# coolo/rl-6-nimmt

Hardware: AMD Instinct MI355X
Metric: env-steps/sec at 65536 concurrent 4-player games, 1/2/4/8 MI355X (higher is better)
Workload: dtype u32; 1 GPU; config2: 65536 x 4-player DrunkHamster self-play per GPU, one episode (10 env-steps) per launch, numpy-MT RNG, int8 obs + actions + rewards + done emitted; games_per_gpu=65536, players=4, env_steps_per_launch=655360, rng=numpy, obs=True, parallelism=dp1 (independent game shards, no data-path collective), launches_per_call=4

## Files before the change

### include/sechs.h

```cpp
#ifndef SECHS_H
#define SECHS_H
#include <stddef.h>
#include <stdint.h>

#ifdef __cplusplus
extern "C" {
#endif

typedef struct sn_env sn_env;

typedef enum {
    SN_OK = 0,
    SN_EINVAL = 1,
    SN_EHIP = 2,
    SN_ENOMEM = 3,
    SN_EUNSUPPORTED = 4,
    SN_ERNG = 5,
} sn_status;

enum {
    SN_RNG_PHILOX = 0,
    SN_RNG_NUMPY_MT = 1,
};

// ... 12 lines not shown
sn_status sn_destroy(sn_env* env);
sn_status sn_info(const sn_env* env, int64_t* num_games, int* num_players, int* num_cards, int* rng_mode);

sn_status sn_reset(sn_env* env, const uint8_t* decks, void* stream);

sn_status sn_reset_to(sn_env* env, const int8_t* board, const int8_t* hands, void* stream);

sn_status sn_step(sn_env* env, const int32_t* actions, int32_t* rewards, uint8_t* done, int32_t* invalid, int flags,
                  void* stream);

sn_status sn_rollout(sn_env* env, int steps, int32_t* rewards, uint8_t* done, uint8_t* actions, int8_t* obs,
                     int obs_stride, int flags, void* stream);

sn_status sn_obs(sn_env* env, void* obs, int dtype, int obs_stride, int flags, void* stream);
sn_status sn_hands(sn_env* env, int8_t* hands, void* stream);
sn_status sn_board(sn_env* env, int8_t* board, void* stream);
sn_status sn_scores(sn_env* env, int32_t* scores, void* stream);
sn_status sn_results(sn_env* env, int32_t* sum_results, int32_t* episodes, void* stream);
sn_status sn_clear_results(sn_env* env, void* stream);

sn_status sn_mt_get(sn_env* env, int64_t game, uint32_t* key_host, int32_t* pos_host);
sn_status sn_mt_set(sn_env* env, int64_t game, const uint32_t* key_host, int32_t pos);
sn_status sn_philox_counter(sn_env* env, int64_t game, uint64_t* counter_host);

int64_t sn_state_bytes(int64_t num_games, int num_players, int rng_mode, int league, int64_t* header_bytes,
                       int64_t* record_bytes);
int64_t sn_state_size(const sn_env* env);
sn_status sn_state_save(sn_env* env, void* blob, int64_t blob_bytes, void* stream);
sn_status sn_state_load(sn_env* env, const void* blob, int64_t blob_bytes, int64_t first, void* stream);

enum { SN_OPT_RING_WORDS = 1, SN_OPT_CHUNK_STEPS = 2, SN_OPT_PIPELINE = 3, SN_OPT_TIMING = 4, SN_OPT_PIPE_GPW = 5,
       SN_OPT_PIPE_LEAD = 6, SN_OPT_PLAY_SPLIT = 7, SN_OPT_PLAY_QUAD = 8, SN_OPT_TWIST_ROUND = 9,
       SN_OPT_TWIST_EVERY = 10, SN_OPT_PIPE_FUSED = 11, SN_OPT_TWIST_SKIP = 12, SN_OPT_PIPE_DEC = 13,
       SN_OPT_TWIST_DEPTH = 14, SN_OPT_PLAY_GROUP = 15, SN_OPT_DEC_WALK = 16, SN_OPT_DEC_EARLY = 17 };
sn_status sn_set_option(sn_env* env, int option, int value);
sn_status sn_pipe_errors(sn_env* env, uint32_t* count);
sn_status sn_kernel_times(sn_env* env, float* play_ms, float* ahead_ms, int32_t* n);
sn_status sn_kernel_times_dec(sn_env* env, float* play_ms, float* ahead_ms, float* decode_ms, int32_t* n);
sn_status sn_debug_phases(uint64_t* out, int n);
sn_status sn_debug_puct_phases(uint64_t* out, int n);
sn_status sn_debug_pipe_words(sn_env* env, int what, int slot, uint32_t* out);
sn_status sn_debug_failures(uint32_t* count, uint32_t* first_line, int selftest);

sn_status sn_step1(sn_env* env, const int32_t* actions_host, int32_t* out_host, int flags);
sn_status sn_reset1(sn_env* env, const uint32_t* key_host, int32_t pos, uint32_t* key_out_host, int32_t* pos_out,
                    int32_t* out_host, int flags);

sn_status sn_league_config(sn_env* env, int num_agents, int min_players, int max_players);
sn_status sn_league_rollout(sn_env* env, int steps, int32_t* rewards, uint8_t* done, uint8_t* actions, int8_t* obs,
                            int obs_stride, int32_t* records, void* stream);
sn_status sn_league_seats(sn_env* env, uint32_t* out, void* stream);

enum { SN_AGENT_RANDOM = 0, SN_AGENT_MCS = 1, SN_AGENT_EXTERNAL = 2 };
sn_status sn_league_agents(sn_env* env, const int32_t* kinds_host, const int32_t* mc_per_card_host,
                           const int32_t* mc_max_host);
sn_status sn_league_step(sn_env* env, const int32_t* actions, int32_t* rewards, int32_t* played, int32_t* records,
                         int32_t* invalid, int32_t* status, void* stream);
sn_status sn_elo_replay(const int32_t* records_host, int64_t num_games, int max_players, int num_agents, double elo_k,
                        double* elos_host);


sn_status sn_mcs_memorize(sn_env* env, uint32_t* avail, int mcs_num_cards, void* stream);

sn_status sn_mcs_rollouts(sn_env* env, const uint32_t* avail, int rollouts, uint64_t seed, uint32_t decision_step,
                          int32_t* sums, void* stream);
sn_status sn_mcs_rollouts_ex(sn_env* env, const uint32_t* avail, int rollouts, uint64_t seed, uint32_t decision_step,
                             int32_t* sums, int32_t* playouts, void* stream);
// ... 101 lines not shown
```

### rl-6-nimmt_amd/csrc/sechs_env.hip

```cpp
#include <hip/hip_runtime.h>

#include <cmath>
#include <cstdio>
#include <cstdlib>
#include <cstring>
#include <new>
#include <string>
#include <type_traits>

#define SECHS_DEBUG_HERE
#include "sechs_state.h"

using namespace sechs;

#include "sechs_reset.h"
#include "sechs_mt_ahead.h"
#include "sechs_play.h"
#include "sechs_decode.h"
#include "sechs_env1.h"
#include "sechs_play_split.h"

template <typename T>
__global__ void k_obs(DevState s, T* out, int stride, int summ) {
    const int64_t i = (int64_t)blockIdx.x * blockDim.x + threadIdx.x;
// ... 127 lines not shown
    DevState& s = e->s;
    s.B = num_games, s.N = num_players, s.C = num_cards, s.rng_mode = rng_mode;
    s.seed = seed, s.game_offset = game_offset;
    const int64_t B = num_games, N = num_players;
    struct {
        void** p;
        size_t bytes;
    } allocs[] = {
        {(void**)&s.hand, sizeof(uint32_t) * N * 3 * B},   {(void**)&s.row_lo, sizeof(uint32_t) * kRows * B},
        {(void**)&s.row_hi, sizeof(uint32_t) * kRows * B}, {(void**)&s.score, sizeof(int32_t) * N * B},
        {(void**)&s.sum_res, sizeof(int32_t) * N * B},     {(void**)&s.episodes, sizeof(int32_t) * B},
        {(void**)&s.mt_pos, sizeof(uint32_t) * B},         {(void**)&s.ctr, sizeof(uint64_t) * B},
        {(void**)&s.mt, rng_mode == SN_RNG_NUMPY_MT ? sizeof(uint32_t) * kMtN * B : 4},
        {(void**)&s.mt0, sizeof(uint32_t) * kMt0Levels * B},
    };
    for (auto& a : allocs) {
        if (hipMalloc(a.p, a.bytes) != hipSuccess) {
            sn_destroy(e);
            return fail(SN_ENOMEM, "hipMalloc of device state failed");
        }
        (void)hipMemset(*a.p, 0, a.bytes);
    }
    e->opt.chunk_steps = 10;
    e->opt.pipe = 1;
    e->opt.pipe_gpw = 64;
    e->opt.pipe_lead = kPipeLead;
    e->phase = -1;
    e->opt.play_split = 1;
    e->opt.twist_round = 1;
    e->opt.twist_every = 4;
    env_default("SECHS_TWIST_EVERY", 1, kTwistEveryMax, e->opt.twist_every);
    e->opt.twist_depth = 3;
    env_default("SECHS_TWIST_DEPTH", 0, kTwistDepthMax, e->opt.twist_depth);
    e->opt.pipe_serial = 0;
    env_default("SECHS_PIPE_SERIAL", 0, 1, e->opt.pipe_serial);
    e->opt.play_group = 1;
    env_default("SECHS_PLAY_GROUP", 0, 1, e->opt.play_group);
    e->opt.dec_walk = 1;
    env_default("SECHS_DEC_WALK", 0, 1, e->opt.dec_walk);
    e->opt.dec_early = 1;
    env_default("SECHS_DEC_EARLY", 0, 1, e->opt.dec_early);
    e->opt.pipe_dec = 1;
    env_default("SECHS_PIPE_DEC", 0, 1, e->opt.pipe_dec);
    if (rng_mode == SN_RNG_NUMPY_MT) {
        struct {
            void** p;
            size_t bytes;
        } pal[] = {{(void**)&s.pring, (size_t)kPipeRing * B},
                   {(void**)&s.pabsc, sizeof(uint32_t) * (kPipeSlots + 2) * B},
                   {(void**)&s.ptend, sizeof(uint32_t) * kPipeSlots * B}, {(void**)&s.ptp, sizeof(uint32_t) * B},
                   {(void**)&s.perr, sizeof(uint32_t)},
                   {(void**)&s.drec, N <= kSplitMaxPlayers ? sizeof(u32x4) * kDecRecords * kDecQuads * B : 16}};
        for (auto& a : pal) {
            if (hipMalloc(a.p, a.bytes) != hipSuccess) {
                sn_destroy(e);
                return fail(SN_ENOMEM, "hipMalloc of the MT pipeline failed");
            }
            (void)hipMemset(*a.p, 0, a.bytes);
        }
        int sysfence = 0;
        env_default("SECHS_EV_SYSFENCE", 0, 1, sysfence);
        const unsigned evf = hipEventDisableTiming | (sysfence ? 0u : (unsigned)hipEventDisableSystemFence);
        if (hipStreamCreateWithFlags(&e->pl.side, hipStreamNonBlocking) != hipSuccess ||
            hipStreamCreateWithFlags(&e->pl.side2, hipStreamNonBlocking) != hipSuccess ||
            hipEventCreateWithFlags(&e->pl.ev_prep2, evf) != hipSuccess ||
            hipEventCreateWithFlags(&e->pl.ev_prep, evf) != hipSuccess ||
            hipEventCreateWithFlags(&e->pl.ev_main, evf) != hipSuccess ||
            hipEventCreateWithFlags(&e->pl.ev_play, evf) != hipSuccess) {
// ... 82 lines not shown
            if (s.ring) (void)hipFree(s.ring);
            s.ring = nullptr;
            s.ring_w = 0;
            if (value) {
                if (hipMalloc((void**)&s.ring, (size_t)value * (size_t)s.B) != hipSuccess) return fail(SN_ENOMEM, "ring allocation failed");
                s.ring_w = value;
            }
            return SN_OK;
        }
        case SN_OPT_CHUNK_STEPS:
            if (value < 1) return fail(SN_EINVAL, "chunk steps must be >= 1");
            e->opt.chunk_steps = value;
            return SN_OK;
        case SN_OPT_PIPELINE:
            if (value != 0 && value != 1) return fail(SN_EINVAL, "pipeline must be 0 or 1");
            e->opt.pipe = value;
            return SN_OK;
        case SN_OPT_PIPE_GPW:
            if (value != 32 && value != 64) return fail(SN_EINVAL, "games per wave must be 32 or 64");
            e->opt.pipe_gpw = value;
            return SN_OK;
        case SN_OPT_PLAY_SPLIT:
            if (value < 0 || value > 1) return fail(SN_EINVAL, "play split must be 0 or 1");
            e->opt.play_split = value;
            return SN_OK;
        case SN_OPT_TWIST_EVERY:
            if (value < 1 || value > kTwistEveryMax) return fail(SN_EINVAL, "twist every must be 1 .. 5");
            e->opt.twist_every = value;
            return SN_OK;
        case SN_OPT_TWIST_DEPTH:
            if (value < 0 || value > kTwistDepthMax) return fail(SN_EINVAL, "twist depth must be 0 .. 3");
            e->opt.twist_depth = value;
            return SN_OK;
        case SN_OPT_TWIST_ROUND:
            if (value < 0 || value > 1) return fail(SN_EINVAL, "twist round must be 0 or 1");
            e->opt.twist_round = value;
            return SN_OK;
        case SN_OPT_PLAY_QUAD:
        case SN_OPT_PIPE_FUSED:
            return fail(SN_EUNSUPPORTED, "option removed (k_play_quad / the fused twist measured slower)");
        case SN_OPT_PIPE_DEC:
            if (value < 0 || value > 1) return fail(SN_EINVAL, "pipe dec must be 0 or 1");
            e->opt.pipe_dec = value;
            return SN_OK;
        case SN_OPT_PLAY_GROUP:
            if (value < 0 || value > 1) return fail(SN_EINVAL, "play group must be 0 or 1");
            e->opt.play_group = value;
            return SN_OK;
        case SN_OPT_DEC_WALK:
            if (value < 0 || value > 1) return fail(SN_EINVAL, "dec walk must be 0 or 1");
            e->opt.dec_walk = value;
            return SN_OK;
        case SN_OPT_DEC_EARLY:
            if (value < 0 || value > 1) return fail(SN_EINVAL, "dec early must be 0 or 1");
            e->opt.dec_early = value;
            return SN_OK;
        case SN_OPT_TWIST_SKIP:
            if (value < 0 || value > 1) return fail(SN_EINVAL, "twist skip must be 0 or 1");
            e->opt.twist_skip = value;
            return SN_OK;
        case SN_OPT_PIPE_LEAD:
            if (value < 64 || value > kPipeLead) return fail(SN_EINVAL, "pipe lead must be in 64..600");
            e->opt.pipe_lead = value;
            return SN_OK;
        case SN_OPT_TIMING:
            if (value < 0 || value > 4096) return fail(SN_EINVAL, "timing launches must be in 0..4096");
// ... 159 lines not shown
        return SN_OK;
    }
    return launch_play_mode(s, a, mode, 64, st);
}

constexpr uint64_t kStartUp = ~0ull;
constexpr uint32_t kSlotMask = (uint32_t)kPipeSlots - 1u;
static inline int pabsc_in(uint64_t p) { return (int)((p + kSlotMask) & kSlotMask); }
static inline int pabsc_out(uint64_t p) { return (int)(p & kSlotMask); }
static inline int ptend_slot(uint64_t G) { return (int)(G & 1u); }
static inline int dec_slot(uint64_t G) { return kDecSlot + (int)(G & 1u); }
static inline int dec_record(int64_t episode) { return (int)(episode % kDecRecords); }

sn_status sn_pipe_sync(sn_env* e, hipStream_t st) {
    if (!e || !e->pl.valid) return SN_OK;
    HIP_TRY(hipStreamWaitEvent(st, e->pl.ev_play, 0));
    HIP_TRY(hipEventRecord(e->pl.ev_prep, e->pl.side));
    HIP_TRY(hipStreamWaitEvent(st, e->pl.ev_prep, 0));
    HIP_TRY(hipEventRecord(e->pl.ev_prep2, e->pl.side2));
    HIP_TRY(hipStreamWaitEvent(st, e->pl.ev_prep2, 0));
    hipLaunchKernelGGL(k_pipe_code, dim3((unsigned)((e->s.B + kBlock / 64 - 1) / (kBlock / 64))), dim3(kBlock), 0, st,
                       e->s, e->pl.pl_cout, e->pl.tw_out);
    HIP_TRY(hipGetLastError());
    e->pl.valid = 0;
    return SN_OK;
}

static int pipe_max_chunk(int N) { return N <= 4 ? 10 : 5; }

static sn_status launch_ahead(const DevState& s, bool init, bool round_tw, const AheadArgs& aa, hipStream_t st) {
    const dim3 pg((unsigned)((s.B + kBlock / 64 - 1) / (kBlock / 64)));
    if (init && round_tw) hipLaunchKernelGGL((k_mt_ahead<true, true>), pg, dim3(kBlock), 0, st, s, aa);
    else if (init) hipLaunchKernelGGL((k_mt_ahead<true, false>), pg, dim3(kBlock), 0, st, s, aa);
    else if (round_tw) hipLaunchKernelGGL((k_mt_ahead<false, true>), pg, dim3(kBlock), 0, st, s, aa);
    else hipLaunchKernelGGL((k_mt_ahead<false, false>), pg, dim3(kBlock), 0, st, s, aa);
    HIP_TRY(hipGetLastError());
    return SN_OK;
}

static sn_status dec_launch(sn_env* e, int64_t e0, int ne, int phi0, int tpar, int cin, int cout, hipStream_t st) {
    const DevState& s = e->s;
    const DecArgs d{dec_record(e0), ne, phi0, tpar, cin, cout};
    const dim3 grid((unsigned)((s.B + kDecBlock - 1) / kDecBlock));
    SN_DISPATCH_N(s.N, {
        if constexpr (NN <= kSplitMaxPlayers) {
            const bool walk = e->opt.dec_walk != 0;
            const bool touch = e->opt.dec_early != 0;
            if (walk && touch) hipLaunchKernelGGL((k_decode<NN, true, true>), grid, dim3(kDecBlock), 0, st, s, d);
            else if (walk) hipLaunchKernelGGL((k_decode<NN, true, false>), grid, dim3(kDecBlock), 0, st, s, d);
            else if (touch) hipLaunchKernelGGL((k_decode<NN, false, true>), grid, dim3(kDecBlock), 0, st, s, d);
            else hipLaunchKernelGGL((k_decode<NN, false, false>), grid, dim3(kDecBlock), 0, st, s, d);
        }
    });
    HIP_TRY(hipGetLastError());
    return SN_OK;
}

static bool dec_ok(const sn_env* e, const PlayArgs& a) {
    return e->opt.pipe_dec && e->phase >= 0 && (a.flags & SN_AUTO_RESET) && !a.actions && !a.invalid && !e->s.lg_K &&
           e->s.N <= kSplitMaxPlayers && e->opt.pipe_gpw == 64 && e->s.drec;
}

static sn_status pipe_start(sn_env* e, int K, bool dec, int lead, hipStream_t st) {
    sn_env::Pipeline& pl = e->pl;
    const AheadArgs aa{dec ? dec_slot(kStartUp - 1) : pabsc_out(kStartUp), ptend_slot(kStartUp - 1), ptend_slot(kStartUp), lead,
                       e->perr_host_dev, dec ? pabsc_out(kStartUp) : -1, e->opt.twist_depth};
    pl.tw_out = ptend_slot(kStartUp), pl.pl_cout = pabsc_out(kStartUp), pl.launches = 0;
    if (const sn_status r = launch_ahead(e->s, true, e->opt.twist_round, aa, st); r != SN_OK) return r;
    if (dec) {
        pl.dec_e = 0;
        const sn_status r = dec_launch(e, 0, K + 1, e->phase, ptend_slot(kStartUp), dec_slot(kStartUp - 1), dec_slot(kStartUp), st);
        if (r != SN_OK) return r;
        pl.dec_next = K + 1;
    }
    HIP_TRY(hipEventRecord(pl.ev_prep, st));
    pl.valid = 1, pl.K = K, pl.dec = dec ? 1 : 0;
    return SN_OK;
}

static sn_status pipe_twist(sn_env* e, uint64_t G, uint64_t p, int64_t e_start, int lead, int ti, hipStream_t st) {
    sn_env::Pipeline& pl = e->pl;
    hipEvent_t* tv = (ti >= 0) ? e->tev + kTimingEvents * ti : nullptr;
    if (e->opt.pipe_serial) HIP_TRY(hipEventRecord(pl.ev_main, st));
    HIP_TRY(hipStreamWaitEvent(pl.side, pl.ev_main, 0));
    if (tv) HIP_TRY(hipEventRecord(tv[2], pl.side));
    const AheadArgs aa{pl.dec ? dec_slot(G - 1) : pabsc_in(p), ptend_slot(G - 1), ptend_slot(G),
                       (e->opt.twist_skip && G >= 1u) ? 0 : lead, e->perr_host_dev, -1, e->opt.twist_depth};
    if (const sn_status r = launch_ahead(e->s, false, e->opt.twist_round, aa, pl.side); r != SN_OK) return r;
    if (tv) HIP_TRY(hipEventRecord(tv[3], pl.side));
    if (pl.dec) {
        const int64_t target = e_start + 2 * pl.K + 1;
        if (e->opt.pipe_serial || G == 0u) HIP_TRY(hipStreamWaitEvent(pl.side2, pl.ev_main, 0));
        if (G >= 1u) HIP_TRY(hipStreamWaitEvent(pl.side2, pl.evt[ptend_slot(G - 1)], 0));
        if (tv) HIP_TRY(hipEventRecord(tv[4], pl.side2));
        const int ne = target > pl.dec_next ? (int)(target - pl.dec_next) : 0;
        const sn_status r = dec_launch(e, pl.dec_next, ne, 0, ptend_slot(G - 1), dec_slot(G - 1), dec_slot(G), pl.side2);
        if (r != SN_OK) return r;
        pl.dec_next = max(pl.dec_next, target);
        if (tv) {
            HIP_TRY(hipEventRecord(tv[5], pl.side2));
            e->tev_tw[ti] |= 2;
        }
        HIP_TRY(hipEventRecord(pl.evd[ptend_slot(G)], pl.side2));
    }
    HIP_TRY(hipEventRecord(pl.evt[ptend_slot(G)], pl.side));
    HIP_TRY(hipEventRecord(pl.ev_prep, pl.side));
    pl.tw_out = ptend_slot(G);
    return SN_OK;
}

static sn_status launch_pipe(sn_env* e, PlayArgs a, LdsPlan plan, hipStream_t st) {
    const DevState& s = e->s;
    sn_env::Pipeline& pl = e->pl;
    const int gpw = e->opt.pipe_gpw, K = e->opt.twist_every;
    const bool dec = dec_ok(e, a);
    const int mode = dec ? RNG_NUMPY_DEC : RNG_NUMPY_PIPE;
    apply_plan(a, dec ? lds_plan(s.N, obs_staged(a.obs, a.obs_stride), RNG_NUMPY_DEC) : plan);
    if (pl.valid && (pl.K != K || (pl.dec != 0) != dec)) {
        if (const sn_status r = sn_pipe_sync(e, st); r != SN_OK) return r;
    }
    const int lead = dec ? min(e->opt.pipe_lead * (K + 1), kPipeRing - kMtN) : e->opt.pipe_lead * K;
    static_assert(kPipeLeadMax <= kPipeRing - kMtN, "the decode-ahead lead is never capped by the ring");
    if (!pl.valid) {
        if (const sn_status r = pipe_start(e, K, dec, lead, st); r != SN_OK) return r;
    } else {
// ... 472 lines not shown
```

### rl-6-nimmt_amd/csrc/sechs_mt_ahead.h

```cpp
#pragma once

constexpr int kPrepGamesPerWave = 4;

template <int NB, int GPW>
__global__ __launch_bounds__(kBlock) void k_mt_prep(DevState s) {
    constexpr uint32_t W = 64u * NB;
    constexpr uint32_t D = kMtN - kMtM;
    const int64_t g0 = ((int64_t)blockIdx.x * (kBlock / 64) + (threadIdx.x >> 6)) * GPW;
    if (g0 >= s.B) return;
    const uint32_t lane = threadIdx.x & 63u;
    uint32_t rem[GPW], KT[GPW], T0[GPW], base[GPW];
    uint32_t A[GPW][NB + 1], C[GPW][NB + 1];
    const uint32_t codes = (lane < (uint32_t)GPW) ? s.mt_pos[min(g0 + (int64_t)lane, s.B - 1)] : 0u;
#pragma unroll
    for (int q = 0; q < GPW; q++) {
        const int64_t g = min(g0 + q, s.B - 1);
        const uint32_t code = __builtin_amdgcn_readlane(codes, q);
        const uint32_t T = code & 0x7FFu;
        rem[q] = (code >> 16) & kMtCntMask;
        const uint32_t add = (rem[q] >= W) ? 0u : ((W - rem[q] + 7u) & ~7u);
        KT[q] = rem[q] + add;
        T0[q] = (T == (uint32_t)kMtN) ? 0u : T;
        base[q] = T0[q] + kMtN - rem[q];
        const uint32_t* st = s.mt + g * kMtN;
// ... 59 lines not shown
                        const uint32_t keep = (1u << (8u * (r + D - k))) - 1u;
                        *dst = (*dst & keep) | (d & ~keep);
                    }
                }
            }
        }
        if (lane == 0u && kt > r) {
            const uint32_t Tn = T0[q] + (kt - r);
            s.mt_pos[g] = ((Tn > (uint32_t)kMtN) ? Tn - kMtN : Tn) | (kt << 16);
        }
    }
}

#ifndef SECHS_NT_OBS
#define SECHS_NT_OBS 1
#endif
#ifndef SECHS_NT_MORE
#define SECHS_NT_MORE 1
#endif
template <class T>
__device__ __forceinline__ void st_nt(T* p, T v, bool nt) {
    if (nt) __builtin_nontemporal_store(v, p);
    else *p = v;
}

struct AheadArgs {
    int cin;
    int tin;
    int tout;
    int lead;
    uint32_t* perr_mirror;
    int cin_copy;
    int depth;
};

__device__ __forceinline__ void mt_round_load(const DevState& s, int64_t G, uint32_t lane, uint32_t (&v)[10]) {
    const uint32_t* st = s.mt + G * kMtN;
#pragma unroll
    for (int k = 0; k < 10; k++) {
        const uint32_t i = 64u * k + lane;
        v[k] = (i < (uint32_t)kMtN) ? st[i] : 0u;
    }
}

__device__ __forceinline__ void mt_round_to_lds(uint32_t lane, uint32_t* w, const uint32_t (&v)[10]) {
#pragma unroll
    for (int k = 0; k < 10; k++) {
        const uint32_t i = 64u * k + lane;
        if (i < (uint32_t)kMtN) w[i] = v[k];
    }
    __builtin_amdgcn_fence(__ATOMIC_SEQ_CST, "wavefront");
}

__device__ __forceinline__ uint32_t mt_twist_lds(uint32_t lane, uint32_t* w) {
    constexpr uint32_t D = kMtN - kMtM;
    const uint32_t old0 = (uint32_t)__builtin_amdgcn_readfirstlane((int)w[0]);
    uint32_t nv[4];
#pragma unroll
    for (int k = 0; k < 4; k++) {
        const uint32_t i = 64u * k + lane;
        nv[k] = (i < D) ? mt_mix(w[i], w[i + 1u], w[i + kMtM]) : 0u;
    }
    __builtin_amdgcn_fence(__ATOMIC_SEQ_CST, "wavefront");
#pragma unroll
    for (int k = 0; k < 4; k++) {
        const uint32_t i = 64u * k + lane;
// ... 24 lines not shown
        if (i < (uint32_t)kMtN) w[i] = nv[k];
    }
    __builtin_amdgcn_fence(__ATOMIC_SEQ_CST, "wavefront");
    return old0;
}

__device__ __forceinline__ void mt_round_emit(const DevState& s, int64_t G, uint32_t lane, const uint32_t* w,
                                              uint32_t te) {
    uint8_t* ring = (uint8_t*)s.pring;
#pragma unroll
    for (int k = 0; k < 3; k++) {
        const uint32_t d = 64u * k + lane;
        if (d < (uint32_t)kMtN / 4u) {
            const u32x4 x = *(const u32x4*)(w + 4u * d);
            const uint32_t y = (mt_temper(x.x) & 0xFFu) | ((mt_temper(x.y) & 0xFFu) << 8) |
                               ((mt_temper(x.z) & 0xFFu) << 16) | ((mt_temper(x.w) & 0xFFu) << 24);
            const uint32_t ri = (te + 4u * d) & (uint32_t)(kPipeRing - 1);
            st_nt((uint32_t*)(ring + ring_byte(ri, G, s.B)), y, SECHS_NT_MORE);
        }
    }
    __builtin_amdgcn_fence(__ATOMIC_SEQ_CST, "wavefront");
}

__device__ __forceinline__ void mt_round_store(const DevState& s, int64_t G, uint32_t lane, const uint32_t* w) {
    uint32_t* st = s.mt + G * kMtN;
#pragma unroll
    for (int k = 0; k < 10; k++) {
        const uint32_t i = 64u * k + lane;
        if (i < (uint32_t)kMtN) st_nt(&st[i], w[i], SECHS_NT_MORE);
    }
    __builtin_amdgcn_fence(__ATOMIC_SEQ_CST, "wavefront");
}

template <bool INIT, bool ROUND = false>
__global__ __launch_bounds__(kBlock) void k_mt_ahead(DevState s, AheadArgs a) {
    constexpr uint32_t D = kMtN - kMtM;
    constexpr uint32_t P1 = 224;
    const int64_t g = (int64_t)blockIdx.x * (kBlock / 64) + (threadIdx.x >> 6);
    if (g >= s.B) return;
    const uint32_t lane = threadIdx.x & 63u;
    const int64_t B = s.B;
    if (g == 0 && lane == 0u && a.perr_mirror)
        __hip_atomic_store(a.perr_mirror, __hip_atomic_load(s.perr, __ATOMIC_RELAXED, __HIP_MEMORY_SCOPE_AGENT),
                           __ATOMIC_RELAXED, __HIP_MEMORY_SCOPE_SYSTEM);
    uint32_t* st = s.mt + g * kMtN;
    uint8_t* ring = (uint8_t*)s.pring;
    uint32_t Tp, t0, c;
    if (INIT) {
        const uint32_t code = s.mt_pos[g];
        Tp = code & 0x7FFu;
        const uint32_t rem = (code >> 16) & kMtCntMask;
        t0 = 0u;
        c = 0u - rem;
        for (uint32_t k0 = 0; k0 < rem; k0 += 64u) {
            const uint32_t k = k0 + lane;
            if (k < rem) {
                const uint32_t v = st[(Tp + kMtN - rem + k) % (uint32_t)kMtN];
                const uint32_t ri = (c + k) & (uint32_t)(kPipeRing - 1);
                ring[ring_byte(ri, g, B)] = (uint8_t)(mt_temper(v) & 0xFFu);
            }
        }
        if (lane == 0u) {
            s.pabsc[(int64_t)a.cin * B + g] = c;
            if (a.cin_copy >= 0) s.pabsc[(int64_t)a.cin_copy * B + g] = c;
        }
    } else {
        Tp = s.ptp[g];
        t0 = s.ptend[(int64_t)a.tin * B + g];
        c = s.pabsc[(int64_t)a.cin * B + g];
    }
    const int32_t lead = (int32_t)(t0 - c);
    if (lead < 0 && lane == 0u) atomicAdd(s.perr, 1u);
    const uint32_t T0 = (Tp == (uint32_t)kMtN) ? 0u : Tp;
    const int32_t lo = a.lead + ((ROUND && INIT) ? kMtN * (int32_t)(g % (int64_t)(a.depth + 1)) : 0);
    const int32_t hi = (ROUND && !INIT) ? a.lead + kMtN * a.depth : lo;
    const bool refill = lead >= 0 && lead < lo;
    const uint32_t n = ROUND ? ((refill && T0 != 0u) ? (uint32_t)kMtN - T0 : 0u)
                             : ((lead >= 0 && lead < a.lead) ? (((uint32_t)(a.lead - lead)) & ~7u) : 0u);
    auto ring_dword = [&](uint32_t j, uint32_t v) {
        const uint32_t y = mt_temper(v) & 0xFFu;
        const uint32_t d = y | (__shfl_down(y, 1) << 8) | (__shfl_down(y, 2) << 16) | (__shfl_down(y, 3) << 24);
        const uint32_t ri = (t0 + j) & (uint32_t)(kPipeRing - 1);
        if ((lane & 3u) == 0u && j < n) st_nt((uint32_t*)(ring + ring_byte(ri, g, B)), d, SECHS_NT_MORE);
    };
    uint32_t ncross = 0u, old0 = 0u;
    auto cross = [&](bool hit, uint32_t old) {
        const uint64_t m = __ballot(hit);
        if (m) {
            const uint32_t v = __shfl(old, (int)__builtin_ctzll(m));
            const uint32_t up = __shfl_up(old0, 1);
            old0 = lane ? up : v;
            ncross++;
        }
    };
    uint32_t A[4] = {0u, 0u, 0u, 0u}, Bv[4], Cv[4], IX[4];
#pragma unroll
    for (int b = 0; b < 4; b++) {
        const uint32_t j = 64u * b + lane;
        IX[b] = 0xFFFFu;
        if (j < n && j < P1) {
            const uint32_t idx = (T0 + j) % (uint32_t)kMtN;
            IX[b] = idx;
            A[b] = st[idx];
            Bv[b] = st[(idx + 1u == (uint32_t)kMtN) ? 0u : idx + 1u];
            Cv[b] = st[(idx < D) ? idx + kMtM : idx - D];
        }
    }
#pragma unroll
// ... 15 lines not shown
        if (j < n) {
            const uint32_t idx = (T0 + j) % (uint32_t)kMtN;
            aa = st[idx];
            v = mt_mix(aa, st[(idx + 1u == (uint32_t)kMtN) ? 0u : idx + 1u], st[(idx < D) ? idx + kMtM : idx - D]);
            st[idx] = v;
            at0 = idx == 0u;
        }
        cross(at0, aa);
        ring_dword(j, v);
    }
    uint32_t Tn = Tp, te = t0 + n;
    if (n) {
        Tn = T0 + n;
        while (Tn > (uint32_t)kMtN) Tn -= kMtN;
    }
    if constexpr (ROUND) {
        if (refill && lead + (int32_t)(te - t0) < hi) {
            __shared__ __attribute__((aligned(16))) uint32_t wround[kBlock / 64][kMtN];
            uint32_t* w = wround[threadIdx.x >> 6];
            __builtin_amdgcn_fence(__ATOMIC_SEQ_CST, "wavefront");
            uint32_t v[10];
            mt_round_load(s, g, lane, v);
            mt_round_to_lds(lane, w, v);
            for (int rr = 0; rr < kMt0Levels - 1 && lead + (int32_t)(te - t0) < hi; rr++) {
                cross(true, mt_twist_lds(lane, w));
                mt_round_emit(s, g, lane, w, te);
                te += kMtN;
            }
            mt_round_store(s, g, lane, w);
            Tn = kMtN;
        }
    }
    SN_DASSERT(ncross <= (uint32_t)kMt0Levels);
    SN_DASSERT(lead < 0 || te - c <= (uint32_t)kPipeSpanMax);
    SN_DASSERT(!ROUND || lead < 0 || te == t0 || (int32_t)(te - c) >= hi);
    SN_DASSERT(!ROUND || te == t0 || Tn == (uint32_t)kMtN);
    if (lane == 0u) {
        s.ptp[g] = Tn;
        s.ptend[(int64_t)a.tout * B + g] = te;
    }
    if (ncross) {
        const uint32_t stk = (lane < (uint32_t)kMt0Levels) ? s.mt0[g * kMt0Levels + lane] : 0u;
        const uint32_t older = __shfl(stk, (int)((lane - ncross) & 63u));
        if (lane < (uint32_t)kMt0Levels) s.mt0[g * kMt0Levels + lane] = (lane < ncross) ? old0 : older;
    }
}

__device__ __forceinline__ uint32_t mt_untwist_y_dev(uint32_t t) {
    const uint32_t lsb = t >> 31;
    return (((lsb ? (t ^ 0x9908b0dfu) : t)) << 1) | lsb;
}

__global__ __launch_bounds__(kBlock) void k_pipe_code(DevState s, int cin, int tin) {
    const int64_t g = (int64_t)blockIdx.x * (kBlock / 64) + (threadIdx.x >> 6);
    if (g >= s.B) return;
    const uint32_t lane = threadIdx.x & 63u;
    int32_t rem = (int32_t)(s.ptend[(int64_t)tin * s.B + g] - s.pabsc[(int64_t)cin * s.B + g]);
    if (rem < 0 && lane == 0u) atomicAdd(s.perr, 1u);
    uint32_t tp = s.ptp[g];
    __shared__ uint32_t sw[kBlock / 64][kMtN], sy[kBlock / 64][kMtN];
    uint32_t* w = sw[threadIdx.x >> 6];
    uint32_t* y = sy[threadIdx.x >> 6];
    uint32_t* a = s.mt + g * kMtN;
    constexpr uint32_t D = kMtN - kMtM;
    int lvl = 0;
    const uint32_t code0 = s.mt_pos[g];
    const bool at0 = code0 == ((uint32_t)kMtN | ((uint32_t)kMtN << 16)) &&
// ... 37 lines not shown
```

### rl-6-nimmt_amd/csrc/sechs_state.h

```cpp
#pragma once
#include <hip/hip_runtime.h>

#include <string>

#include "../../include/sechs.h"
#include "sechs_device.h"

namespace sechs {

struct DevState {
    int64_t B;
    int N, C, rng_mode, pad_;
    uint64_t seed, game_offset;
    uint32_t* hand;
    uint32_t* row_lo;
    uint32_t* row_hi;
    int32_t* score;
    int32_t* sum_res;
    int32_t* episodes;
    uint32_t* mt;
    uint32_t* mt_pos;
    uint64_t* ctr;
    uint32_t* mt0;
    u32x4* ring;
// ... 2 lines not shown
    u32x4* pring;
    uint32_t* pabsc;
    uint32_t* ptend;
    uint32_t* ptp;
    uint32_t* perr;
    u32x4* drec;
    uint32_t* lgs;
    int lg_K, lg_lo, lg_hi, lg_pad;
    uint32_t* lmem;
    int32_t* lpc;
    int32_t* lpf;
};

constexpr int kMt0Levels = 16;
constexpr int kPipeSlots = 8;
constexpr int kDecSlot = kPipeSlots;
constexpr int kDecRecords = 16;
constexpr int kDecQuads = 6;
constexpr int kTimingEvents = 6;
constexpr int kPipeRing = 8192;

__host__ __device__ __forceinline__ int64_t ring16(uint32_t u, int64_t g, int64_t B) {
    u &= (uint32_t)(kPipeRing / 16 - 1);
    return ((int64_t)(u >> 2) * B + g) * 4 + (u & 3u);
}
__host__ __device__ __forceinline__ int64_t ring_byte(uint32_t ri, int64_t g, int64_t B) {
    return ring16(ri >> 4, g, B) * 16 + (ri & 15u);
}

constexpr int kPipeLead = 600;
constexpr int kPipeWin = 240;

constexpr int kTwistEveryMax = 5, kTwistDepthMax = 3;
static_assert((kPipeSlots & (kPipeSlots - 1)) == 0, "pabsc / ptend slots are taken mod kPipeSlots with a mask");
static_assert(kPipeSlots >= kTwistEveryMax + 3, "no play launch overwrites a pabsc slot a running twist reads");
static_assert(kDecRecords >= 3 * kTwistEveryMax + 1, "no decode overwrites a record a running play launch reads");
constexpr int kPipeLeadMax = kPipeLead * (kTwistEveryMax + 1);
constexpr int kPipeSpanMax = kPipeLeadMax + kMtN * kTwistDepthMax + kMtN - 1;
static_assert(kPipeSpanMax + 64 <= kPipeRing && (kPipeRing & (kPipeRing - 1)) == 0, "pring holds the twisted span");
constexpr int kPipeSyncSpanMax = 296 * (2 * kTwistEveryMax + 1) + kPipeSpanMax;
static_assert(kPipeSyncSpanMax / kMtN <= kMt0Levels, "mt0 holds every round k_pipe_code may undo");
static_assert((kPipeSpanMax + kMtN - 1) / kMtN < kMt0Levels, "k_mt_ahead's round loop reaches the start-up lead");

constexpr int kBlock = 256;
constexpr int kLeagueMaxPlayers = 6;
constexpr int kLeagueMaxAgents = 16;
constexpr int kSplitMaxPlayers = 4;
constexpr int kSplitEarly = 2;
constexpr int kDeckStride = 108;
constexpr int kDealStride = 212;

template <int MODE, int PF = 1>
struct RngOf;
template <int PF>
struct RngOf<RNG_NUMPY_MT, PF> {
    using T = MtGenT<PF>;
    static __device__ __forceinline__ void load(const DevState& s, int64_t g, T& r, ByteBuf& buf) {
        r.load(s.mt + g * kMtN, s.mt_pos[g], buf);
    }
    static __device__ __forceinline__ void store(const DevState& s, int64_t g, T& r, const ByteBuf& buf) {
        s.mt_pos[g] = r.save(buf);
    }
};
template <int PF>
struct RngOf<RNG_PHILOX, PF> {
    using T = PhiloxGen;
    static __device__ __forceinline__ void load(const DevState& s, int64_t g, T& r, ByteBuf& buf) {
        r.load((uint32_t)s.seed, (uint32_t)(s.seed >> 32), s.game_offset + (uint64_t)g, s.ctr[g], buf);
    }
    static __device__ __forceinline__ void store(const DevState& s, int64_t g, const T& r, const ByteBuf& buf) {
        s.ctr[g] = r.consumed(buf);
// ... 704 lines not shown
        case 1: { constexpr int NN = 1; BODY; } break;                                   \
        case 2: { constexpr int NN = 2; BODY; } break;                                   \
        case 3: { constexpr int NN = 3; BODY; } break;                                   \
        case 4: { constexpr int NN = 4; BODY; } break;                                   \
        case 5: { constexpr int NN = 5; BODY; } break;                                   \
        case 6: { constexpr int NN = 6; BODY; } break;                                   \
        case 7: { constexpr int NN = 7; BODY; } break;                                   \
        case 8: { constexpr int NN = 8; BODY; } break;                                   \
        case 9: { constexpr int NN = 9; BODY; } break;                                   \
        case 10: { constexpr int NN = 10; BODY; } break;                                 \
        default: return ::sechs::set_error(SN_EINVAL, "num_players out of range");      \
    }
#endif

}

struct sn_env {
    int device;
    int cus;
    int lg_phase;
    int lg_kind[16];
    int lg_mpc[16], lg_mmax[16];
    int phase;
    struct Options {
        int chunk_steps;
        int pipe;
        int pipe_gpw;
        int pipe_lead;
        int pipe_dec;
        int play_group;
        int dec_walk;
        int dec_early;
        int pipe_serial;
        int play_split;
        int twist_every;
        int twist_round;
        int twist_depth;
        int twist_skip;
    } opt;
    sechs::DevState s;
    struct Pipeline {
        int valid;
        int K, dec;
        uint64_t launches;
        int tw_out;
        int pl_cout;
        int64_t dec_e;
        int64_t dec_next;
        hipStream_t side, side2;
        hipEvent_t evt[2];
        hipEvent_t evd[2], ev_prep2;
        hipEvent_t ev_prep, ev_main, ev_play;
    } pl;
    uint32_t* perr_host;
    uint32_t* perr_host_dev;
    uint32_t* hbuf;
    uint32_t* hbuf_dev;
    hipEvent_t* tev;
    int* tev_tw;
    int tcap, tn;
};

extern "C" sn_status sn_pipe_sync(sn_env* e, hipStream_t st);
```

### rl-6-nimmt_amd/rl_6_nimmt/_native.py

```python
import ctypes
import os

import torch

_PKG_ROOT = os.path.dirname(os.path.dirname(os.path.abspath(__file__)))
LIB_PATH = os.environ.get("SECHS_LIB", os.path.join(_PKG_ROOT, "libsechs.so"))

SN_OK, SN_EINVAL, SN_EHIP, SN_ENOMEM, SN_EUNSUPPORTED, SN_ERNG = 0, 1, 2, 3, 4, 5
SN_RNG_PHILOX, SN_RNG_NUMPY_MT = 0, 1
SN_I8, SN_I16, SN_I32, SN_I64, SN_F32 = 1, 2, 3, 4, 5
SN_AUTO_RESET, SN_NO_SUMMARIES = 1, 2
SN_OPT_RING_WORDS, SN_OPT_CHUNK_STEPS, SN_OPT_PIPELINE, SN_OPT_TIMING, SN_OPT_PIPE_GPW, SN_OPT_PIPE_LEAD = 1, 2, 3, 4, 5, 6
SN_OPT_PLAY_SPLIT = 7
SN_OPT_TWIST_ROUND = 9
SN_OPT_TWIST_EVERY = 10
SN_OPT_TWIST_SKIP = 12
SN_OPT_PIPE_DEC = 13
SN_OPT_TWIST_DEPTH = 14
SN_OPT_PLAY_GROUP = 15
SN_OPT_DEC_WALK = 16
SN_OPT_DEC_EARLY = 17
SN_AGENT_RANDOM, SN_AGENT_MCS, SN_AGENT_EXTERNAL = 0, 1, 2

class SnPuct(ctypes.Structure):

    _fields_ = [
        ("seats_mask", ctypes.c_uint32),
        ("n", ctypes.c_int),
        ("puct_root", ctypes.c_int),
        ("c_puct", ctypes.c_double),
        ("seed", ctypes.c_uint64),
        ("step", ctypes.c_uint32),
        ("rollout", ctypes.c_uint32),
        ("avail", ctypes.c_void_p),
        ("rollouts", ctypes.c_void_p),
        ("stats", ctypes.c_void_p),
        ("hist", ctypes.c_void_p),
        ("root_probs", ctypes.c_void_p),
        ("step_dev", ctypes.c_void_p),
        ("dec_list", ctypes.c_void_p),
        ("num_dec", ctypes.c_int64),
        ("logit_stride", ctypes.c_int32),
        ("logit_bf16", ctypes.c_int32),
    ]


class SnDqnGpow(ctypes.Structure):

    _fields_ = [("v", ctypes.c_double * 10)]


_P = ctypes.c_void_p
_I = ctypes.c_int
_I64 = ctypes.c_int64
# ... 136 lines not shown
```

### rl-6-nimmt_amd/rl_6_nimmt/vec_env.py

```python
import ctypes

import numpy as np
import torch

from . import _native as nat

RNG_MODES = {"philox": nat.SN_RNG_PHILOX, "numpy": nat.SN_RNG_NUMPY_MT}
ROWS, THRESHOLD, HAND = 4, 6, 10


def obs_length(include_summaries=True):
    return 10 + 1 + (3 * ROWS if include_summaries else 0) + ROWS * THRESHOLD


class VecSechsNimmtEnv:
    def __init__(self, num_games, num_players=4, num_cards=104, seed=0, game_offset=0, rng="numpy", device=None,
                 include_summaries=True):
        nat.require_gpu()
        if rng not in RNG_MODES:
            raise ValueError(f"rng must be one of {sorted(RNG_MODES)}")
        if device is None:
            idx = torch.cuda.current_device()
        else:
            d = torch.device(device)
# ... 94 lines not shown
        o = self._empty((self.num_games, self.num_players, stride), dtype)
        nat.check(nat.lib().sn_obs(self._h, nat.ptr(o), self._DT[dtype], stride, self._flags(), self._stream()), "sn_obs")
        return o

    def hands(self):
        h = self._empty((self.num_games, self.num_players, HAND), torch.int8)
        nat.check(nat.lib().sn_hands(self._h, nat.ptr(h), self._stream()), "sn_hands")
        return h

    def board(self):
        b = self._empty((self.num_games, ROWS, THRESHOLD), torch.int8)
        nat.check(nat.lib().sn_board(self._h, nat.ptr(b), self._stream()), "sn_board")
        return b

    def scores(self):
        s = self._empty((self.num_games, self.num_players), torch.int32)
        nat.check(nat.lib().sn_scores(self._h, nat.ptr(s), self._stream()), "sn_scores")
        return s

    def results(self):
        s = self._empty((self.num_games, self.num_players), torch.int32)
        e = self._empty((self.num_games,), torch.int32)
        nat.check(nat.lib().sn_results(self._h, nat.ptr(s), nat.ptr(e), self._stream()), "sn_results")
        return s, e

    def clear_results(self):
        nat.check(nat.lib().sn_clear_results(self._h, self._stream()), "sn_clear_results")

    _OPTIONS = (
        ("pipe_lead", nat.SN_OPT_PIPE_LEAD, int), ("pipe_gpw", nat.SN_OPT_PIPE_GPW, int),
        ("play_split", nat.SN_OPT_PLAY_SPLIT, int), ("twist_every", nat.SN_OPT_TWIST_EVERY, int),
        ("twist_round", nat.SN_OPT_TWIST_ROUND, int), ("twist_depth", nat.SN_OPT_TWIST_DEPTH, int),
        ("play_group", nat.SN_OPT_PLAY_GROUP, int), ("walk_draws", nat.SN_OPT_DEC_WALK, int),
        ("dec_early", nat.SN_OPT_DEC_EARLY, int),
        ("pipe_dec", nat.SN_OPT_PIPE_DEC, int), ("twist_skip", nat.SN_OPT_TWIST_SKIP, int),
        ("pipeline", nat.SN_OPT_PIPELINE, lambda v: int(bool(v))), ("ring_words", nat.SN_OPT_RING_WORDS, int),
        ("chunk_steps", nat.SN_OPT_CHUNK_STEPS, int),
    )

    def set_option(self, ring_words=None, chunk_steps=None, pipeline=None, pipe_gpw=None, pipe_lead=None,
                   play_split=None, twist_round=None, twist_every=None, twist_skip=None, pipe_dec=None,
                   twist_depth=None, play_group=None, walk_draws=None, dec_early=None):
        given = locals()
        for name, opt, conv in self._OPTIONS:
            if given[name] is not None:
                nat.check(nat.lib().sn_set_option(self._h, opt, conv(given[name])), "sn_set_option")

    def time_kernels(self, launches):
        nat.check(nat.lib().sn_set_option(self._h, nat.SN_OPT_TIMING, int(launches)), "sn_set_option")

    def kernel_times(self, with_decode=False):
        a, b, c, n = ctypes.c_float(), ctypes.c_float(), ctypes.c_float(), ctypes.c_int32()
        nat.check(nat.lib().sn_kernel_times_dec(self._h, ctypes.byref(a), ctypes.byref(b), ctypes.byref(c),
                                                ctypes.byref(n)), "sn_kernel_times_dec")
        return (a.value, b.value, c.value, n.value) if with_decode else (a.value, b.value, n.value)

    def pipe_errors(self):
        c = ctypes.c_uint32()
        nat.check(nat.lib().sn_pipe_errors(self._h, ctypes.byref(c)), "sn_pipe_errors")
        return c.value

    def get_mt_state(self, game=0):
        key = np.zeros(624, dtype=np.uint32)
        pos = ctypes.c_int32()
        torch.cuda.current_stream(self.device).synchronize()
        nat.check(nat.lib().sn_mt_get(self._h, game, key.ctypes.data_as(ctypes.c_void_p), ctypes.byref(pos)), "sn_mt_get")
        return key, int(pos.value)

    def set_mt_state(self, key, pos, game=0):
        key = np.ascontiguousarray(key, dtype=np.uint32)
        assert key.shape == (624,)
        torch.cuda.current_stream(self.device).synchronize()
        nat.check(nat.lib().sn_mt_set(self._h, game, key.ctypes.data_as(ctypes.c_void_p), int(pos)), "sn_mt_set")

    def snapshot(self):
# ... 26 lines not shown
```

Measured before the change: 12.23 billion env-steps/s.

## Jitter per-game MT twist thresholds and let twist wait on decode event directly

Adds a per-game hash jitter to the whole-round Mersenne Twister refill threshold, plus a staggered steady-state dispatch on the first pipelined launch. The aim is to spread twist work evenly across launches instead of having many games twist in the same launch. It also makes the side-stream twist wait on the previous decode event rather than the main-stream event, so it can overlap more with play. In exchange the ring span grows by up to one MT state, and the cross-stream dependency ordering changes, which raises correctness risk.

Measured after the change: 10.18 billion env-steps/s. 16.8% lower.

```diff
diff --git a/include/sechs.h b/include/sechs.h
--- a/include/sechs.h
+++ b/include/sechs.h
@@ -68,7 +68,8 @@
 enum { SN_OPT_RING_WORDS = 1, SN_OPT_CHUNK_STEPS = 2, SN_OPT_PIPELINE = 3, SN_OPT_TIMING = 4, SN_OPT_PIPE_GPW = 5,
        SN_OPT_PIPE_LEAD = 6, SN_OPT_PLAY_SPLIT = 7, SN_OPT_PLAY_QUAD = 8, SN_OPT_TWIST_ROUND = 9,
        SN_OPT_TWIST_EVERY = 10, SN_OPT_PIPE_FUSED = 11, SN_OPT_TWIST_SKIP = 12, SN_OPT_PIPE_DEC = 13,
-       SN_OPT_TWIST_DEPTH = 14, SN_OPT_PLAY_GROUP = 15, SN_OPT_DEC_WALK = 16, SN_OPT_DEC_EARLY = 17 };
+       SN_OPT_TWIST_DEPTH = 14, SN_OPT_PLAY_GROUP = 15, SN_OPT_DEC_WALK = 16, SN_OPT_DEC_EARLY = 17,
+       SN_OPT_TWIST_JITTER = 18 };
 sn_status sn_set_option(sn_env* env, int option, int value);
 sn_status sn_pipe_errors(sn_env* env, uint32_t* count);
 sn_status sn_kernel_times(sn_env* env, float* play_ms, float* ahead_ms, int32_t* n);
diff --git a/rl-6-nimmt_amd/csrc/sechs_env.hip b/rl-6-nimmt_amd/csrc/sechs_env.hip
--- a/rl-6-nimmt_amd/csrc/sechs_env.hip
+++ b/rl-6-nimmt_amd/csrc/sechs_env.hip
@@ -183,8 +183,12 @@
     env_default("SECHS_TWIST_EVERY", 1, kTwistEveryMax, e->opt.twist_every);
     e->opt.twist_depth = 3;
     env_default("SECHS_TWIST_DEPTH", 0, kTwistDepthMax, e->opt.twist_depth);
+    e->opt.twist_jitter = 1;
+    env_default("SECHS_TWIST_JITTER", 0, 1, e->opt.twist_jitter);
     e->opt.pipe_serial = 0;
     env_default("SECHS_PIPE_SERIAL", 0, 1, e->opt.pipe_serial);
+    e->opt.twist_direct = 1;
+    env_default("SECHS_TWIST_DIRECT", 0, 1, e->opt.twist_direct);
     e->opt.play_group = 1;
     env_default("SECHS_PLAY_GROUP", 0, 1, e->opt.play_group);
     e->opt.dec_walk = 1;
@@ -333,6 +337,10 @@
             if (value < 0 || value > kTwistDepthMax) return fail(SN_EINVAL, "twist depth must be 0 .. 3");
             e->opt.twist_depth = value;
             return SN_OK;
+        case SN_OPT_TWIST_JITTER:
+            if (value < 0 || value > 1) return fail(SN_EINVAL, "twist jitter must be 0 or 1");
+            e->opt.twist_jitter = value;
+            return SN_OK;
         case SN_OPT_TWIST_ROUND:
             if (value < 0 || value > 1) return fail(SN_EINVAL, "twist round must be 0 or 1");
             e->opt.twist_round = value;
@@ -558,6 +566,7 @@
     const dim3 pg((unsigned)((s.B + kBlock / 64 - 1) / (kBlock / 64)));
     if (init && round_tw) hipLaunchKernelGGL((k_mt_ahead<true, true>), pg, dim3(kBlock), 0, st, s, aa);
     else if (init) hipLaunchKernelGGL((k_mt_ahead<true, false>), pg, dim3(kBlock), 0, st, s, aa);
+    else if (round_tw && aa.stagger) hipLaunchKernelGGL((k_mt_ahead<false, true, true>), pg, dim3(kBlock), 0, st, s, aa);
     else if (round_tw) hipLaunchKernelGGL((k_mt_ahead<false, true>), pg, dim3(kBlock), 0, st, s, aa);
     else hipLaunchKernelGGL((k_mt_ahead<false, false>), pg, dim3(kBlock), 0, st, s, aa);
     HIP_TRY(hipGetLastError());
@@ -587,10 +596,12 @@
            e->s.N <= kSplitMaxPlayers && e->opt.pipe_gpw == 64 && e->s.drec;
 }
 
+static inline int jitter_on(const sn_env* e) { return (e->opt.twist_jitter && e->opt.twist_round && !e->opt.twist_skip) ? 1 : 0; }
+
 static sn_status pipe_start(sn_env* e, int K, bool dec, int lead, hipStream_t st) {
     sn_env::Pipeline& pl = e->pl;
     const AheadArgs aa{dec ? dec_slot(kStartUp - 1) : pabsc_out(kStartUp), ptend_slot(kStartUp - 1), ptend_slot(kStartUp), lead,
-                       e->perr_host_dev, dec ? pabsc_out(kStartUp) : -1, e->opt.twist_depth};
+                       e->perr_host_dev, dec ? pabsc_out(kStartUp) : -1, e->opt.twist_depth, jitter_on(e), 0};
     pl.tw_out = ptend_slot(kStartUp), pl.pl_cout = pabsc_out(kStartUp), pl.launches = 0;
     if (const sn_status r = launch_ahead(e->s, true, e->opt.twist_round, aa, st); r != SN_OK) return r;
     if (dec) {
@@ -604,19 +615,24 @@
     return SN_OK;
 }
 
+static inline bool twist_direct(const sn_env* e, uint64_t G) {
+    return e->pl.dec && G >= 1u && e->opt.twist_direct && !e->opt.pipe_serial;
+}
+
 static sn_status pipe_twist(sn_env* e, uint64_t G, uint64_t p, int64_t e_start, int lead, int ti, hipStream_t st) {
     sn_env::Pipeline& pl = e->pl;
     hipEvent_t* tv = (ti >= 0) ? e->tev + kTimingEvents * ti : nullptr;
     if (e->opt.pipe_serial) HIP_TRY(hipEventRecord(pl.ev_main, st));
-    HIP_TRY(hipStreamWaitEvent(pl.side, pl.ev_main, 0));
+    HIP_TRY(hipStreamWaitEvent(pl.side, twist_direct(e, G) ? pl.evd[ptend_slot(G - 1)] : pl.ev_main, 0));
     if (tv) HIP_TRY(hipEventRecord(tv[2], pl.side));
     const AheadArgs aa{pl.dec ? dec_slot(G - 1) : pabsc_in(p), ptend_slot(G - 1), ptend_slot(G),
-                       (e->opt.twist_skip && G >= 1u) ? 0 : lead, e->perr_host_dev, -1, e->opt.twist_depth};
+                       (e->opt.twist_skip && G >= 1u) ? 0 : lead, e->perr_host_dev, -1, e->opt.twist_depth,
+                       jitter_on(e), (pl.dec && G == 0u && jitter_on(e)) ? 1 : 0};
     if (const sn_status r = launch_ahead(e->s, false, e->opt.twist_round, aa, pl.side); r != SN_OK) return r;
     if (tv) HIP_TRY(hipEventRecord(tv[3], pl.side));
     if (pl.dec) {
         const int64_t target = e_start + 2 * pl.K + 1;
-        if (e->opt.pipe_serial || G == 0u) HIP_TRY(hipStreamWaitEvent(pl.side2, pl.ev_main, 0));
+        if (e->opt.pipe_serial || G == 0u || twist_direct(e, G)) HIP_TRY(hipStreamWaitEvent(pl.side2, pl.ev_main, 0));
         if (G >= 1u) HIP_TRY(hipStreamWaitEvent(pl.side2, pl.evt[ptend_slot(G - 1)], 0));
         if (tv) HIP_TRY(hipEventRecord(tv[4], pl.side2));
         const int ne = target > pl.dec_next ? (int)(target - pl.dec_next) : 0;
diff --git a/rl-6-nimmt_amd/csrc/sechs_mt_ahead.h b/rl-6-nimmt_amd/csrc/sechs_mt_ahead.h
--- a/rl-6-nimmt_amd/csrc/sechs_mt_ahead.h
+++ b/rl-6-nimmt_amd/csrc/sechs_mt_ahead.h
@@ -115,6 +115,8 @@
     uint32_t* perr_mirror;
     int cin_copy;
     int depth;
+    int jitter;
+    int stagger;
 };
 
 __device__ __forceinline__ void mt_round_load(const DevState& s, int64_t G, uint32_t lane, uint32_t (&v)[10]) {
@@ -205,8 +207,9 @@
     __builtin_amdgcn_fence(__ATOMIC_SEQ_CST, "wavefront");
 }
 
-template <bool INIT, bool ROUND = false>
+template <bool INIT, bool ROUND = false, bool STAG = false>
 __global__ __launch_bounds__(kBlock) void k_mt_ahead(DevState s, AheadArgs a) {
+    static_assert(!STAG || (ROUND && !INIT), "only a steady whole-round dispatch staggers again");
     constexpr uint32_t D = kMtN - kMtM;
     constexpr uint32_t P1 = 224;
     const int64_t g = (int64_t)blockIdx.x * (kBlock / 64) + (threadIdx.x >> 6);
@@ -245,8 +248,11 @@
     const int32_t lead = (int32_t)(t0 - c);
     if (lead < 0 && lane == 0u) atomicAdd(s.perr, 1u);
     const uint32_t T0 = (Tp == (uint32_t)kMtN) ? 0u : Tp;
-    const int32_t lo = a.lead + ((ROUND && INIT) ? kMtN * (int32_t)(g % (int64_t)(a.depth + 1)) : 0);
-    const int32_t hi = (ROUND && !INIT) ? a.lead + kMtN * a.depth : lo;
+    const uint32_t gu = (uint32_t)__builtin_amdgcn_readfirstlane((int)(uint32_t)g);
+    const int32_t jit = (ROUND && a.jitter && a.lead > 0) ? (int32_t)twist_jitter((int64_t)gu) : 0;
+    constexpr bool stag = ROUND && (INIT || STAG);
+    const int32_t lo = a.lead + jit + (stag ? kMtN * (int32_t)(gu % (uint32_t)(a.depth + 1)) : 0);
+    const int32_t hi = (ROUND && !stag) ? lo + kMtN * a.depth : lo;
     const bool refill = lead >= 0 && lead < lo;
     const uint32_t n = ROUND ? ((refill && T0 != 0u) ? (uint32_t)kMtN - T0 : 0u)
                              : ((lead >= 0 && lead < a.lead) ? (((uint32_t)(a.lead - lead)) & ~7u) : 0u);
@@ -328,7 +334,11 @@
         }
     }
     SN_DASSERT(ncross <= (uint32_t)kMt0Levels);
+    SN_DASSERT(jit >= 0 && jit <= kTwistJitterMax && (jit == 0 || (ROUND && a.jitter && a.lead > 0)));
+    SN_DASSERT(STAG == (a.stagger != 0));
     SN_DASSERT(lead < 0 || te - c <= (uint32_t)kPipeSpanMax);
+    SN_DASSERT(!ROUND || lead < 0 || te == t0 || (int32_t)(te - c) < hi + kMtN);
+    SN_DASSERT(!ROUND || lead < 0 || te != t0 || lead >= lo);
     SN_DASSERT(!ROUND || lead < 0 || te == t0 || (int32_t)(te - c) >= hi);
     SN_DASSERT(!ROUND || te == t0 || Tn == (uint32_t)kMtN);
     if (lane == 0u) {
diff --git a/rl-6-nimmt_amd/csrc/sechs_state.h b/rl-6-nimmt_amd/csrc/sechs_state.h
--- a/rl-6-nimmt_amd/csrc/sechs_state.h
+++ b/rl-6-nimmt_amd/csrc/sechs_state.h
@@ -58,11 +58,16 @@
 constexpr int kPipeWin = 240;
 
 constexpr int kTwistEveryMax = 5, kTwistDepthMax = 3;
+constexpr int kTwistJitterMax = kMtN - 1;
+__host__ __device__ __forceinline__ uint32_t twist_jitter(int64_t g) {
+    const uint32_t x = (uint32_t)g * 0x9E3779B1u;
+    return (uint32_t)(((uint64_t)x * (uint32_t)kMtN) >> 32);
+}
 static_assert((kPipeSlots & (kPipeSlots - 1)) == 0, "pabsc / ptend slots are taken mod kPipeSlots with a mask");
 static_assert(kPipeSlots >= kTwistEveryMax + 3, "no play launch overwrites a pabsc slot a running twist reads");
 static_assert(kDecRecords >= 3 * kTwistEveryMax + 1, "no decode overwrites a record a running play launch reads");
 constexpr int kPipeLeadMax = kPipeLead * (kTwistEveryMax + 1);
-constexpr int kPipeSpanMax = kPipeLeadMax + kMtN * kTwistDepthMax + kMtN - 1;
+constexpr int kPipeSpanMax = kPipeLeadMax + kTwistJitterMax + kMtN * kTwistDepthMax + kMtN - 1;
 static_assert(kPipeSpanMax + 64 <= kPipeRing && (kPipeRing & (kPipeRing - 1)) == 0, "pring holds the twisted span");
 constexpr int kPipeSyncSpanMax = 296 * (2 * kTwistEveryMax + 1) + kPipeSpanMax;
 static_assert(kPipeSyncSpanMax / kMtN <= kMt0Levels, "mt0 holds every round k_pipe_code may undo");
@@ -833,10 +838,12 @@
         int dec_walk;
         int dec_early;
         int pipe_serial;
+        int twist_direct;
         int play_split;
         int twist_every;
         int twist_round;
         int twist_depth;
+        int twist_jitter;
         int twist_skip;
     } opt;
     sechs::DevState s;
diff --git a/rl-6-nimmt_amd/rl_6_nimmt/_native.py b/rl-6-nimmt_amd/rl_6_nimmt/_native.py
--- a/rl-6-nimmt_amd/rl_6_nimmt/_native.py
+++ b/rl-6-nimmt_amd/rl_6_nimmt/_native.py
@@ -20,6 +20,7 @@
 SN_OPT_PLAY_GROUP = 15
 SN_OPT_DEC_WALK = 16
 SN_OPT_DEC_EARLY = 17
+SN_OPT_TWIST_JITTER = 18
 SN_AGENT_RANDOM, SN_AGENT_MCS, SN_AGENT_EXTERNAL = 0, 1, 2
 
 class SnPuct(ctypes.Structure):
diff --git a/rl-6-nimmt_amd/rl_6_nimmt/vec_env.py b/rl-6-nimmt_amd/rl_6_nimmt/vec_env.py
--- a/rl-6-nimmt_amd/rl_6_nimmt/vec_env.py
+++ b/rl-6-nimmt_amd/rl_6_nimmt/vec_env.py
@@ -150,7 +150,7 @@
         ("play_split", nat.SN_OPT_PLAY_SPLIT, int), ("twist_every", nat.SN_OPT_TWIST_EVERY, int),
         ("twist_round", nat.SN_OPT_TWIST_ROUND, int), ("twist_depth", nat.SN_OPT_TWIST_DEPTH, int),
         ("play_group", nat.SN_OPT_PLAY_GROUP, int), ("walk_draws", nat.SN_OPT_DEC_WALK, int),
-        ("dec_early", nat.SN_OPT_DEC_EARLY, int),
+        ("dec_early", nat.SN_OPT_DEC_EARLY, int), ("twist_jitter", nat.SN_OPT_TWIST_JITTER, int),
         ("pipe_dec", nat.SN_OPT_PIPE_DEC, int), ("twist_skip", nat.SN_OPT_TWIST_SKIP, int),
         ("pipeline", nat.SN_OPT_PIPELINE, lambda v: int(bool(v))), ("ring_words", nat.SN_OPT_RING_WORDS, int),
         ("chunk_steps", nat.SN_OPT_CHUNK_STEPS, int),
@@ -158,7 +158,7 @@
 
     def set_option(self, ring_words=None, chunk_steps=None, pipeline=None, pipe_gpw=None, pipe_lead=None,
                    play_split=None, twist_round=None, twist_every=None, twist_skip=None, pipe_dec=None,
-                   twist_depth=None, play_group=None, walk_draws=None, dec_early=None):
+                   twist_depth=None, play_group=None, walk_draws=None, dec_early=None, twist_jitter=None):
         given = locals()
         for name, opt, conv in self._OPTIONS:
             if given[name] is not None:
```
